# Hebbalali/dgp-toolbox

Measured on NVIDIA B200. Metric: DGP ELBO+grad point-samples/s, higher is better.
Workload: dtype f64

## Files before the change

### dgp_toolbox_b200/csrc/common.cuh

```cuda
#pragma once
#include <cuda_runtime.h>
#include <cstdint>
#include <type_traits>
#include <cstdio>
#include <string>

#define DGP_OK 0
#define DGP_ERR_CUDA -1
#define DGP_ERR_ARG -2
#define DGP_ERR_UNSUPPORTED -3
#define DGP_ERR_NUMERIC -4

namespace dgp {

constexpr int kTileM = 64;
constexpr int kTileP = 128;
constexpr int kMaxD = 32;

__host__ __device__ inline long round_up(long x, long m) { return (x + m - 1) / m * m; }

__device__ __forceinline__ void dmma884(double& c0, double& c1, double a, double b) {
  asm volatile("mma.sync.aligned.m8n8k4.row.col.f64.f64.f64.f64 {%0,%1},{%2},{%3},{%0,%1};"
               : "+d"(c0), "+d"(c1) : "d"(a), "d"(b));
}

__device__ __forceinline__ void cp_async16(void* smem, const void* gmem) {
  unsigned s = (unsigned)__cvta_generic_to_shared(smem);
  asm volatile("cp.async.cg.shared.global [%0], [%1], 16;" ::"r"(s), "l"(gmem));
}
__device__ __forceinline__ void cp_async8(void* smem, const void* gmem) {
  unsigned s = (unsigned)__cvta_generic_to_shared(smem);
  asm volatile("cp.async.ca.shared.global [%0], [%1], 8;" ::"r"(s), "l"(gmem));
}
__device__ __forceinline__ void cp_async_commit() { asm volatile("cp.async.commit_group;"); }
template <int N>
__device__ __forceinline__ void cp_async_wait() { asm volatile("cp.async.wait_group %0;" ::"n"(N)); }

__device__ __forceinline__ double exp_nonpos(double x) {
  const double xc = fmax(x, -700.0);
  double t = fma(xc, 1.4426950408889634074, 6755399441055744.0);
  const int n = __double2loint(t);
  t -= 6755399441055744.0;
  double r = fma(t, -6.93147180369123816490e-01, xc);
  r = fma(t, -1.90821492927058770002e-10, r);
  double p = 1.6059043836821613e-10;
  p = fma(p, r, 2.08767569878681e-09);
  p = fma(p, r, 2.505210838544172e-08);
  p = fma(p, r, 2.755731922398589e-07);
  p = fma(p, r, 2.7557319223985893e-06);
  p = fma(p, r, 2.48015873015873e-05);
  p = fma(p, r, 1.984126984126984e-04);
  p = fma(p, r, 1.388888888888889e-03);
  p = fma(p, r, 8.333333333333333e-03);
  p = fma(p, r, 4.1666666666666664e-02);
  p = fma(p, r, 1.6666666666666666e-01);
  p = fma(p, r, 0.5);
  p = fma(p, r, 1.0);
  p = fma(p, r, 1.0);
  const double y = __hiloint2double(__double2hiint(p) + (n << 20), __double2loint(p));
  return x != x ? x : y;
}

__device__ __forceinline__ void kernel_eval(int kind, double r2, double s2, double& k, double& gfac) {
  if (kind == 0) {
    k = s2 * exp_nonpos(-0.5 * r2);
    gfac = k;
  } else if (kind == 1) {
    const double a = 1.7320508075688772935;
    const double r = sqrt(fmax(r2, 1e-36)), e = exp_nonpos(-a * r);
    k = s2 * (1.0 + a * r) * e;
// ... 36 lines not shown
```

### dgp_toolbox_b200/csrc/dgp_b200.cu

```cuda
#include "../../include/dgp_b200.h"

#include <dlfcn.h>

#include <cmath>
#include <cstdlib>
#include <cstring>
#include <string>
#include <vector>

#include "acq.cuh"
#include "common.cuh"
#include "fused.cuh"
#include "fused_bwd.cuh"
#include "fullcov.cuh"
#include "extk.cuh"
#include "compkern.cuh"
#include "gemm.cuh"
#include "layer.cuh"
#include "philox.cuh"
#include "prep.cuh"
#include "small.cuh"

using namespace dgp;

// ... 284 lines not shown
    const long ctas = p.tiles * s;
    const long waves = (ctas + p.slots - 1) / p.slots;
    const double eff = (double)ctas / (double)(waves * p.slots);
    if (eff > best_eff + 0.02) { best_eff = eff; best = (int)s; }
  }
  return best;
}

template <typename F>
int dispatch_dmax(int D, F&& f) {
  if (D <= 1) return f(std::integral_constant<int, 1>());
  if (D <= 2) return f(std::integral_constant<int, 2>());
  if (D <= 4) return f(std::integral_constant<int, 4>());
  if (D <= 8) return f(std::integral_constant<int, 8>());
  if (D <= 16) return f(std::integral_constant<int, 16>());
  return f(std::integral_constant<int, 32>());
}

int check_layer(dgp_ctx* c, const dgp_layer_desc& L) {
  if (L.D_in < 1 || L.D_in > kMaxD - 1 || L.D_out < 1 || L.D_out > kMaxD || L.M < 1) {
    c->err = "layer widths must satisfy 1 <= D_in <= 31, 1 <= D_out <= 32, M >= 1";
    return DGP_ERR_ARG;
  }
  if (round_up(L.M, kTileM) > 768) { c->err = "M > 768 is not supported by the single-CTA Cholesky"; return DGP_ERR_UNSUPPORTED; }
  if (L.kernel_kind < 0 || L.kernel_kind > 2) { c->err = "kernel_kind must be 0 (SquaredExponential), 1 (Matern32) or 2 (Matern52)"; return DGP_ERR_UNSUPPORTED; }
  if (L.mean_kind < 0 || L.mean_kind > 2) { c->err = "mean_kind must be 0 (Zero), 1 (Identity) or 2 (Linear)"; return DGP_ERR_ARG; }
  if (L.mean_kind == 1 && L.D_in != L.D_out) { c->err = "Identity mean function needs D_in == D_out"; return DGP_ERR_ARG; }
  if (L.mean_kind == 2 && !L.mf_W) { c->err = "Linear mean function needs mf_W"; return DGP_ERR_ARG; }
  if (!L.Z || !L.lengthscales || !L.variance || !L.q_mu || !L.q_sqrt) { c->err = "null parameter pointer in layer descriptor"; return DGP_ERR_ARG; }
  return DGP_OK;
}

struct LayerWs {
  int M = 0, Mp = 0, D_in = 0, D_out = 0;
  double *Ku = nullptr, *Knj = nullptr, *L = nullptr, *Linv = nullptr, *LinvT = nullptr;
  double *RpT = nullptr, *Rcat = nullptr, *qmuP = nullptr;
  double *Kinv = nullptr, *alpha = nullptr, *KRcat = nullptr, *LRcat = nullptr, *KSK = nullptr;
  double *dKu = nullptr, *dR = nullptr, *dqmu = nullptr, *H = nullptr, *rbf_red = nullptr, *sgv = nullptr;
  double *dZk = nullptr, *kuu_part = nullptr, *kuu_red = nullptr, *kl = nullptr;
  double *Zs = nullptr, *zz = nullptr, *stream = nullptr;
  PanelDesc* sched = nullptr;
  int NP = 0, fcfg = -1;
  bool vform = false;
  bool white = false;
  double *Cmat = nullptr, *betaP = nullptr;
  double *CTcat = nullptr, *G1 = nullptr, *DCt = nullptr, *Wacc = nullptr, *dbeta = nullptr, *dqmu2 = nullptr, *dRcat = nullptr;
  double *dLinv = nullptr, *sq1 = nullptr, *sq2 = nullptr;
  double* bstream = nullptr; int bcfg = -1, NPb = 0;
  double* part_small = nullptr;
};

struct FusedChoice { int BM, PT; };
constexpr FusedChoice kFusedChoices[4] = {{128, 64}, {128, 32}, {64, 64}, {64, 32}};
constexpr size_t kMaxSmem = 227 * 1024;

size_t fused_smem(int cfg, int Mp, int D_in, int D_out) {
  switch (cfg) {
    case 0: return FusedCfg<128, 64, 4, 2>::smem_bytes(Mp, D_in, D_out);
    case 1: return FusedCfg<128, 32, 4, 2>::smem_bytes(Mp, D_in, D_out);
    case 2: return FusedCfg<64, 64, 2, 4>::smem_bytes(Mp, D_in, D_out);
    default: return FusedCfg<64, 32, 2, 4>::smem_bytes(Mp, D_in, D_out);
  }
}

int pick_fused_cfg(int Mp, int D_in, int D_out) {
  static const char* force = getenv("DGP_B200_FUSED_CFG");
  if (force) { const int cfg = atoi(force); if (cfg >= 0 && cfg < 4 && Mp % kFusedChoices[cfg].BM == 0 && fused_smem(cfg, Mp, D_in, D_out) <= kMaxSmem) return cfg; }
  for (int cfg = 0; cfg < 4; ++cfg) {
    if (Mp % kFusedChoices[cfg].BM) continue;
    if (fused_smem(cfg, Mp, D_in, D_out) <= kMaxSmem) return cfg;
  }
  return -1;
}

constexpr int kFusedBwdBM[2] = {128, 64};
size_t fused_bwd_smem(int cfg, int Mp, int D_in, int D_out) {
  return cfg == 0 ? FusedBwdCfg<128, 64, 4, 2>::smem_bytes(Mp, D_in, D_out) : FusedBwdCfg<64, 64, 2, 4>::smem_bytes(Mp, D_in, D_out);
}
int pick_fused_bwd_cfg(int Mp, int D_in, int D_out) {
  if (D_in > 16) return -1;
  static const char* force = getenv("DGP_B200_FUSED_BWD_CFG");
  for (int cfg = force ? atoi(force) : 0; cfg < 2; ++cfg) {
    if (cfg < 0 || Mp % kFusedBwdBM[cfg]) continue;
    if (fused_bwd_smem(cfg, Mp, D_in, D_out) <= kMaxSmem) return cfg;
  }
  return -1;
}

std::vector<PanelDesc> build_schedule(int Mp, int BM, int D_out, bool vform) {
  std::vector<PanelDesc> v;
  const int nb = Mp / BM, kpb = BM / kPanelK, kt = Mp / kPanelK;
  for (int i = nb - 1; i >= 0; --i)
    for (int ks = 0; ks < (i + 1) * kpb; ++ks) {
      int fl = (ks == 0 ? kPanelFirst : 0) | (ks == (i + 1) * kpb - 1 ? kPanelLast : 0) | (ks * kPanelK >= i * BM ? kPanelClip : 0);
      if ((fl & kPanelLast) && i == 0) fl |= kPanelStageEnd;
      v.push_back(PanelDesc{0, 0, i, ks * kPanelK, fl, 0});
    }
  auto upper = [&](int kind, int d0, int nd) {
    for (int i = 0; i < nb; ++i)
      for (int ks = i * kpb; ks < kt; ++ks) {
        int fl = (ks == i * kpb ? kPanelFirst : 0) | (ks == kt - 1 ? kPanelLast : 0) | (ks * kPanelK < (i + 1) * BM ? kPanelClip : 0);
        if ((fl & kPanelLast) && i == nb - 1) fl |= kPanelStageEnd;
        for (int d = d0; d < d0 + nd; ++d) v.push_back(PanelDesc{kind, d, i, ks * kPanelK, fl, 0});
      }
  };
  if (!vform) upper(1, 0, 1);
  for (int dp = 0; dp < D_out / 2; ++dp) upper(2, 2 * dp, 2);
  if (D_out & 1) upper(2, D_out - 1, 1);
  return v;
}

enum PrepLevel { PREP_FWD = 0, PREP_KL = 1, PREP_GRAD = 2 };

struct LayerPath { bool fused, vform; };

LayerPath ctx_path(const dgp_ctx* c, PrepLevel level, long point_samples) {
  const bool vform = level == PREP_FWD ? c->vform_forward_calls
                                       : level == PREP_GRAD && c->use_vform_grad && point_samples >= c->vform_grad_min_ps;
  return {c->use_fused, vform};
}

int chol_smem_optin(dgp_ctx* c) {
  if (c->chol_configured) return DGP_OK;
  CK(cudaFuncSetAttribute(chol_inv_kernel, cudaFuncAttributeMaxDynamicSharedMemorySize, (int)chol_smem_bytes(768)));
  CK(cudaFuncSetAttribute(tri_inv_kernel, cudaFuncAttributeMaxDynamicSharedMemorySize, (int)tri_inv_smem_bytes(768)));
  c->chol_configured = true;
  return DGP_OK;
}

void split_long_k(GemmArgs& g, int D, double* part) {
// ... 333 lines not shown
  CAT(DGP_CAT_RBF_BWD);
  RbfBwdArgs r;
  memset(&r, 0, sizeof(r));
  r.W = W; r.A = A; r.gq = up.gq; r.Gbar = Gbar; r.Xin = cl.Xin; r.xmod = cl.xmod; r.Z = d.Z; r.ls = d.lengthscales;
  r.var = d.variance; r.M = w.M; r.Mp = w.Mp; r.D_in = w.D_in; r.P = P; r.Pp = Pp; r.Gm = up.Gm; r.D_out = w.D_out;
  r.mean_kind = d.mean_kind; r.mfW = d.mf_W; r.kind = d.kernel_kind; r.dXin = dXin; r.XaugPad = XaugPad; r.part = rbf_part;
  const bool small = Pp / 128 < 2L * c->num_sms && rbf_bwd_smem_bytes(w.M, w.D_in) <= kRbfBwdSmemMax;
  nb = small ? Pp / kRbfCols : Pp / 128;
  const size_t smem = small ? rbf_bwd_smem_bytes(w.M, w.D_in) : ((size_t)w.M * w.D_in + kMaxD + 32) * sizeof(double);
  return dispatch_dmax(w.D_in, [&](auto dm) -> int {
    constexpr int DM = decltype(dm)::value;
    if (small) {
      if (!c->dry) CK(cudaFuncSetAttribute((rbf_bwd2d_kernel<DM, VF>), cudaFuncAttributeMaxDynamicSharedMemorySize, (int)kRbfBwdSmemMax));
      LAUNCH((rbf_bwd2d_kernel<DM, VF>), (unsigned)nb, 256, smem, r);
    } else {
      if (!c->dry) CK(cudaFuncSetAttribute((rbf_bwd_kernel<DM, VF>), cudaFuncAttributeMaxDynamicSharedMemorySize, (int)kRbfBwdSmemMax));
      LAUNCH((rbf_bwd_kernel<DM, VF>), (unsigned)nb, 128, smem, r);
    }
    return DGP_OK;
  });
}

int backward_layer(dgp_ctx* c, const dgp_layer_desc& d, const LayerWs& w, const ChunkLayer& cl, const Temps& tmp,
                   const Upstream& up, double* dXin, double* XaugPad, double* rbf_part, const ParamScratch& ps, long Nc, long S, bool first_chunk,
                   bool params = true) {
  const long P = Nc * S, Pp = round_up(P, kTileP);
  const int Mp = w.Mp, D = w.D_out;
  const double beta = first_chunk ? 0.0 : 1.0;
  double* dA = tmp.t0;
  double* W = tmp.t1;
  double* Gbar = tmp.t2;
  if (w.vform) {
    const double* V = cl.A;
    double* dV = dA;
    double* Kbar = W;
    const bool fused_bwd = w.bcfg >= 0;
    const long ntile64 = Pp / 64;
    long nbv = 0;
    if (fused_bwd) {
      CAT(DGP_CAT_FUSED_BWD);
      FusedBwdArgs f;
      memset(&f, 0, sizeof(f));
      f.stream = w.bstream; f.V = V; f.T = cl.T; f.GvT = up.GvT; f.gq = up.gq; f.Gm = up.GmPad; f.gm_ld = 32; f.beta = w.betaP;
      f.Zs = w.Zs; f.zz = w.zz; f.ls = d.lengthscales; f.var = d.variance; f.Xin = cl.Xin; f.xmod = cl.xmod; f.D_in = w.D_in;
      f.mfW = d.mf_W; f.mean_kind = d.mean_kind; f.kind = d.kernel_kind; f.M = w.M; f.Mp = Mp; f.D_out = D; f.P = P; f.Pp = Pp;
      f.dV = nullptr;
      f.Gbar = Gbar; f.dXin = dXin; f.XaugPad = XaugPad; f.part = rbf_part;
      f.warp_major_groups = c->warp_major_groups ? 1 : 0; f.group_skew = c->group_skew;
      nbv = ntile64 * (w.bcfg == 0 ? 2 : 4);
      const size_t smem = fused_bwd_smem(w.bcfg, Mp, w.D_in, D);
      const unsigned grid = (unsigned)(ntile64 < c->num_sms ? ntile64 : c->num_sms);
#define FUSED_BWD_LAUNCH(BM_, WM_, WN_, DM_)                                                                                \
      do {                                                                                                                  \
        if (!c->dry) CK(cudaFuncSetAttribute((fused_backward_kernel<BM_, 64, WM_, WN_, DM_>), cudaFuncAttributeMaxDynamicSharedMemorySize, (int)kMaxSmem)); \
        LAUNCH((fused_backward_kernel<BM_, 64, WM_, WN_, DM_>), grid, 384, smem, f);                                        \
      } while (0)
      if (w.bcfg == 0) { if (w.D_in <= 8) FUSED_BWD_LAUNCH(128, 4, 2, 8); else FUSED_BWD_LAUNCH(128, 4, 2, 16); }
      else { if (w.D_in <= 8) FUSED_BWD_LAUNCH(64, 2, 4, 8); else FUSED_BWD_LAUNCH(64, 2, 4, 16); }
#undef FUSED_BWD_LAUNCH
    } else {
    CAT(DGP_CAT_GEMM_BWD_DATA);
    GemmArgs g = gargs(w.betaP, 32, up.GmPad, 32, dV, Pp, Mp, (int)Pp, 32);
    RC(gemm(c, g, true));
    g = gargs(w.CTcat, (long)D * Mp, cl.T, Pp, dV, Pp, Mp, (int)Pp, D * Mp);
    g.a_tri = 1; g.kblocks = D; g.kblk = Mp; g.bscale = up.GvT; g.ld_bscale = Pp; g.bscale_mul = 2.0; g.beta = 1.0;
    if (D == 1) g.kblocks = 1;
    g.epi_plane = V; g.ld_epi = Pp; g.epi_col = up.gq; g.epi_mul = 2.0;
    RC(gemm(c, g, false));
    g = gargs(w.LinvT, Mp, dV, Pp, Kbar, Pp, Mp, (int)Pp, Mp);
    g.a_tri = 2;
    RC(gemm(c, g, false));
    RC(kernel_adjoint<true>(c, d, w, cl, up, Kbar, nullptr, Gbar, dXin, XaugPad, rbf_part, P, nbv));
    }
    if (!params) return DGP_OK;
    CAT(DGP_CAT_GEMM_BWD_PARAM);
    GemmArgs pg[3];
    const bool pnt[3] = {true, false, false};
    const int slots[3] = {1, 2, 3};
    pg[0] = gargs(V, Pp, V, Pp, w.Wacc, (long)D * Mp, Mp, Mp, (int)Pp);
    pg[0].alpha = 2.0; pg[0].beta = beta; pg[0].batch = D; pg[0].sA = 0; pg[0].sB = 0; pg[0].sC = Mp; pg[0].c_lower = 1;
    pg[0].kscale = up.GvT; pg[0].sScale = Pp;
    pg[1] = gargs(V, Pp, up.GmPad, 32, w.dbeta, 32, Mp, 32, (int)Pp);
    pg[1].beta = beta;
    pg[2] = gargs(Gbar, Pp, XaugPad, 32, w.H, 32, Mp, 32, (int)Pp);
    pg[2].beta = beta;
    RC(param_gemms(c, pg, pnt, 3, ps, slots, [&]() -> int {
      LAUNCH(reduce_partials_kernel, w.D_in + 1, 256, 0, rbf_part, nbv, w.D_in + 1, w.rbf_red, first_chunk ? 0 : 1);
      LAUNCH(reduce_partials_kernel, 3, 256, 0, up.part, up.nblocks, 3, w.sgv, first_chunk ? 0 : 1);
      return DGP_OK;
    }));
    return DGP_OK;
  }
  CAT(DGP_CAT_GEMM_BWD_DATA);
  RC(aform_adjoint(c, w, cl.T, up.GmPad, up.GvT, dA, W, Pp, &ps));
  long nb = 0;
  RC(kernel_adjoint<false>(c, d, w, cl, up, W, cl.A, Gbar, dXin, XaugPad, rbf_part, P, nb));
  if (!params) return DGP_OK;
  CAT(DGP_CAT_GEMM_BWD_PARAM);
  GemmArgs pg[4];
  const bool pnt[4] = {kAformParamNT[0], kAformParamNT[1], kAformParamNT[2], false};
  aform_param_args(w, W, cl.A, cl.T, up.GvT, up.GmPad, Pp, beta, pg);
  pg[3] = gargs(Gbar, Pp, XaugPad, 32, w.H, 32, Mp, 32, (int)Pp);
  pg[3].beta = beta;
  RC(param_gemms(c, pg, pnt, 4, ps, nullptr, [&]() -> int {
    LAUNCH(reduce_partials_kernel, w.D_in + 1, 256, 0, rbf_part, nb, w.D_in + 1, w.rbf_red, first_chunk ? 0 : 1);
    LAUNCH(reduce_partials_kernel, 3, 256, 0, up.part, up.nblocks, 3, w.sgv, first_chunk ? 0 : 1);
    return DGP_OK;
  }));
// ... 1565 lines not shown
```

### dgp_toolbox_b200/csrc/fused_bwd.cuh

```cuda
#pragma once
#include "common.cuh"
#include "fused.cuh"

namespace dgp {

struct FusedBwdArgs {
  const double* stream;
  const double* V; const double* T;
  const double* GvT; const double* gq;
  const double* Gm; int gm_ld;
  const double* beta;
  const double* Zs; const double* ls; const double* var;
  const double* Xin; long xmod; int D_in;
  const double* mfW; int mean_kind; int kind;
  int M, Mp, D_out; long P, Pp;
  double* dV; double* Gbar;
  double* dXin;
  double* XaugPad;
  double* part;
  int warp_major_groups, group_skew;
  const double* zz;
};

__host__ __device__ __forceinline__ int zigzag(int idx, int n) { return (idx & 1) ? n - 1 - (idx >> 1) : (idx >> 1); }

template <int BM>
__global__ void __launch_bounds__(256) pack_bwd_stream_kernel(const double* __restrict__ Cmat, const double* __restrict__ LinvT,
                                                              int Mp, int D, double* __restrict__ stream) {
  const int nb = Mp / BM, kpb = BM / kPanelK;
  int q = blockIdx.x, pass = 0, i = 0, d = 0, ks = 0;
  const int NP0 = D * kpb * nb * (nb + 1) / 2;
  if (q < NP0) {
    for (i = 0;; ++i) { const int cnt = D * (i + 1) * kpb; if (q < cnt) break; q -= cnt; }
    d = q / ((i + 1) * kpb); ks = zigzag(q % ((i + 1) * kpb), (i + 1) * kpb);
  } else {
    q -= NP0; pass = 1;
    for (i = 0;; ++i) { const int cnt = (nb - i) * kpb; if (q < cnt) break; q -= cnt; }
    ks = i * kpb + zigzag(q, (nb - i) * kpb);
  }
  double* dst = stream + (long)blockIdx.x * BM * kPanelK;
  for (int idx = threadIdx.x; idx < BM * kPanelK; idx += blockDim.x) {
    const int r = idx % BM, k = idx / BM;
    const int row = i * BM + r, col = ks * kPanelK + k;
    dst[panel_swz(r, k)] = pass == 0 ? Cmat[((long)d * Mp + col) * Mp + row] : LinvT[(long)row * Mp + col];
  }
}

template <int LO, int HI, int TM, int TN, int WM, int LDT, bool SC>
__device__ __forceinline__ void bwd_panel_block(double (&c0)[TM][TN], double (&c1)[TM][TN], const double* __restrict__ pan,
                                                const double* __restrict__ bt, const double (&sc)[TN], int wm, int g8, int t4) {
#pragma unroll
  for (int kk = 0; kk < 4; ++kk) {
    double bv[TN], av[HI - LO > 0 ? HI - LO : 1];
#pragma unroll
    for (int j = 0; j < TN; ++j) bv[j] = bt[kk * 4 * LDT + j * 8];
#pragma unroll
    for (int i = LO; i < HI; ++i) {
      const int row = i * 8 * WM + wm * 8 + g8;
      av[i - LO] = pan[row * kPanelK + (((kk ^ (row & 3)) << 2) | t4)];
    }
    if (SC) {
#pragma unroll
      for (int j = 0; j < TN; ++j) bv[j] *= sc[j];
    }
#pragma unroll
    for (int i = LO; i < HI; ++i)
#pragma unroll
      for (int j = 0; j < TN; ++j) dmma884(c0[i][j], c1[i][j], av[i - LO], bv[j]);
  }
}
template <int TM, int TN, int WM, int LDT, bool SC>
__device__ __forceinline__ void bwd_panel_dispatch(double (&c0)[TM][TN], double (&c1)[TM][TN], const double* pan, const double* bt,
                                                   const double (&sc)[TN], int wm, int g8, int t4, int lo, int hi) {
  static_assert(TM <= 4, "dispatch covers TM <= 4");
  if (lo == 0) {
    if (hi == TM) { bwd_panel_block<0, TM, TM, TN, WM, LDT, SC>(c0, c1, pan, bt, sc, wm, g8, t4); return; }
    if constexpr (TM >= 2) { if (hi == 1) { bwd_panel_block<0, 1, TM, TN, WM, LDT, SC>(c0, c1, pan, bt, sc, wm, g8, t4); return; } }
    if constexpr (TM >= 3) { if (hi == 2) { bwd_panel_block<0, 2, TM, TN, WM, LDT, SC>(c0, c1, pan, bt, sc, wm, g8, t4); return; } }
    if constexpr (TM >= 4) { if (hi == 3) { bwd_panel_block<0, 3, TM, TN, WM, LDT, SC>(c0, c1, pan, bt, sc, wm, g8, t4); return; } }
    return;
  }
  if constexpr (TM >= 2) { if (lo == TM - 1) { bwd_panel_block<TM - 1, TM, TM, TN, WM, LDT, SC>(c0, c1, pan, bt, sc, wm, g8, t4); return; } }
  if constexpr (TM >= 3) { if (lo == TM - 2) { bwd_panel_block<TM - 2, TM, TM, TN, WM, LDT, SC>(c0, c1, pan, bt, sc, wm, g8, t4); return; } }
  if constexpr (TM >= 4) { if (lo == TM - 3) { bwd_panel_block<TM - 3, TM, TM, TN, WM, LDT, SC>(c0, c1, pan, bt, sc, wm, g8, t4); return; } }
}



template <int BM, int PT, int WM, int WN>
struct FusedBwdCfg {
  static_assert(WM * WN == 8, "8 consumer warps");
  static constexpr int THREADS = 384;
  static constexpr int GT = WM * 32, GC = PT / WN;
  static constexpr int TM = BM / (8 * WM), TN = GC / 8;
  static constexpr int LDT = PT + 4;
  static constexpr int PANEL = BM * kPanelK, SLAB = kPanelK * LDT, STAGE = PANEL + SLAB;
  static constexpr int STAGES = 3;
  static size_t smem_bytes(int Mp, int D_in, int D_out) {
    return ((size_t)STAGES * STAGE + (size_t)Mp * LDT + (size_t)D_in * PT + (size_t)D_out * PT + (size_t)PT + 2 * STAGES + 2 + (size_t)WN * WM * (kMaxD + 1) + (size_t)PT * (D_in + 1)) * sizeof(double);
  }
};

template <int BM, int PT, int WM, int WN, int DMAX>
__global__ void __launch_bounds__(384, 1) fused_backward_kernel(FusedBwdArgs a) {
  using Cfg = FusedBwdCfg<BM, PT, WM, WN>;
  constexpr int TM = Cfg::TM, TN = Cfg::TN, LDT = Cfg::LDT, PANEL = Cfg::PANEL, STAGE = Cfg::STAGE, STAGES = Cfg::STAGES;
  constexpr int GT = Cfg::GT, GC = Cfg::GC, KPB = BM / kPanelK;
  constexpr int XSW = GC == 32 ? 1 : 0;
  extern __shared__ __align__(128) double bsmem[];
  double* pbuf = bsmem;
  double* tile = pbuf + STAGES * STAGE;
  double* xs_all = tile + (size_t)a.Mp * LDT;
  double* gv2_all = xs_all + a.D_in * PT;
  double* gq_all = gv2_all + a.D_out * PT;
  unsigned long long* full = reinterpret_cast<unsigned long long*>(gq_all + PT);
  unsigned long long* empty = full + STAGES;
  unsigned long long* vbar = empty + STAGES;
  double* red_all = reinterpret_cast<double*>(vbar + 2);
  double* us_all = red_all + WN * WM * (kMaxD + 1);

  const int tid = threadIdx.x, lane = tid & 31, warp = tid >> 5;
  const int nb = a.Mp / BM, kt = a.Mp / kPanelK;
  const int ntiles = (int)(a.Pp / PT);
  const int my_tiles = (int)blockIdx.x < ntiles ? (ntiles - (int)blockIdx.x + (int)gridDim.x - 1) / (int)gridDim.x : 0;

  if (tid == 0) {
    for (int s = 0; s < STAGES; ++s) { mbar_init(full + s, 1); mbar_init(empty + s, 8); }
    mbar_init(vbar, 1);
    asm volatile("fence.mbarrier_init.release.cluster;" ::: "memory");
  }
  __syncthreads();

  if (warp >= 8) {
    regs_shrink();
    if (warp > 8) return;
    if (lane == 0) {
      int st = 0;
      unsigned ph = 0;
#ifndef DGP_BWD_AHEAD
#define DGP_BWD_AHEAD 8
#endif
      constexpr int kAhead = DGP_BWD_AHEAD;
      int f_tl = 0, f_i = 0, f_d = 0, f_ks = 0;
      auto prefetch_next = [&]() {
        if (f_tl >= my_tiles) return;
        const double* trow = a.T + ((long)f_d * a.Mp + (long)zigzag(f_ks, (f_i + 1) * KPB) * kPanelK) * a.Pp + (long)(blockIdx.x + f_tl * gridDim.x) * PT;
#pragma unroll 4
        for (int r = 0; r < kPanelK; ++r)
          asm volatile("cp.async.bulk.prefetch.L2.global [%0], %1;" ::"l"(trow + (long)r * a.Pp), "r"(PT * 8) : "memory");
        if (++f_ks == (f_i + 1) * KPB) { f_ks = 0; if (++f_d == a.D_out) { f_d = 0; if (++f_i == nb) { f_i = 0; ++f_tl; } } }
      };
      for (int q = 0; q < kAhead; ++q) prefetch_next();
      for (int tl = 0; tl < my_tiles; ++tl) {
        const long p0 = (long)(blockIdx.x + tl * gridDim.x) * PT;
        const double* src = a.stream;
        int issued = 0;
        for (int i = 0; i < nb; ++i)
          for (int d = 0; d < a.D_out; ++d)
            for (int ksi = 0; ksi < (i + 1) * KPB; ++ksi) {
              const int ks = zigzag(ksi, (i + 1) * KPB);
              mbar_wait(empty + st, ph ^ 1);
              if (issued++ == STAGES) {
                mbar_arrive_expect_tx(vbar, (unsigned)(a.Mp * PT * 8));
                for (int r = 0; r < a.Mp; ++r) bulk_g2s(tile + r * LDT, a.V + (long)r * a.Pp + p0, PT * 8, vbar);
              }
              double* dst = pbuf + st * STAGE;
#ifdef DGP_BWD_EXPERIMENT_NO_SLABS
              mbar_arrive_expect_tx(full + st, PANEL * 8);
              bulk_g2s(dst, src, PANEL * 8, full + st);
#else
              const int r0 = max(0, ks * kPanelK - i * BM);
              mbar_arrive_expect_tx(full + st, (unsigned)(((BM - r0) * kPanelK + kPanelK * PT) * 8));
              bulk_g2s(dst + r0 * kPanelK, src + r0 * kPanelK, (unsigned)((BM - r0) * kPanelK * 8), full + st);
              const double* trow = a.T + ((long)d * a.Mp + (long)ks * kPanelK) * a.Pp + p0;
#pragma unroll 4
              for (int r = 0; r < kPanelK; ++r) bulk_g2s(dst + PANEL + r * LDT, trow + (long)r * a.Pp, PT * 8, full + st);
#endif
              prefetch_next();
              src += PANEL;
              if (++st == STAGES) { st = 0; ph ^= 1; }
            }
        for (int i = 0; i < nb; ++i)
          for (int ksi = 0; ksi < kt - i * KPB; ++ksi) {
            const int ks = i * KPB + zigzag(ksi, kt - i * KPB);
            mbar_wait(empty + st, ph ^ 1);
            const int nr = min(BM, ks * kPanelK - i * BM + kPanelK);
            mbar_arrive_expect_tx(full + st, (unsigned)(nr * kPanelK * 8));
            bulk_g2s(pbuf + st * STAGE, src, (unsigned)(nr * kPanelK * 8), full + st);
            src += PANEL;
            if (++st == STAGES) { st = 0; ph ^= 1; }
          }
      }
    }
    return;
  }

  regs_grow();
  const int g8 = lane >> 2, t4 = lane & 3;
  const int wm = a.warp_major_groups ? warp % WM : warp / WN, wn = a.warp_major_groups ? warp / WM : warp % WN;
  const int tg = wm * 32 + lane;
  const int col0 = wn * GC;
  double* xs = xs_all + wn * a.D_in * GC;
  double* gv2 = gv2_all + wn * a.D_out * GC;
  double* gqs = gq_all + wn * GC;
  double* red = red_all + wn * WM * (kMaxD + 1);
  double* us = us_all + wn * GC * (a.D_in + 1);
  const int bar_id = 1 + wn;
  const double s2 = a.var[0];
  int cst = 0;
  unsigned cph = 0;
  double c0[TM][TN], c1[TM][TN];

  if (a.group_skew > 0 && wn > 0) {
    const long long t0 = clock64();
    while (clock64() - t0 < (long long)a.group_skew * wn) {}
  }
#ifdef DGP_DEBUG_PHASECLK
  long long ph_pro = 0, ph_p0 = 0, ph_be = 0, ph_p1 = 0, ph_row = 0, ph_red = 0, ph_out = 0, ph_wait = 0;
  const long long ph_t0 = clock64();
#endif
  for (int tl = 0; tl < my_tiles; ++tl) {
    const long tile_index = (long)blockIdx.x + (long)tl * gridDim.x;
    const long p0 = tile_index * PT + col0;
    PH_MARK(ph_a);
    group_sync(bar_id, GT);
    for (int idx = tg; idx < a.D_in * GC; idx += GT) {
      const int j = idx / GC, c = idx % GC;
      const long p = p0 + c;
      xs[j * GC + (c ^ (XSW * ((j & 3) << 3)))] = (p < a.P) ? a.Xin[(p % a.xmod) * a.D_in + j] * (1.0 / a.ls[j]) : 0.0;
    }
    for (int idx = tg; idx < a.D_out * GC; idx += GT) {
      const int d = idx / GC, c = idx % GC;
      gv2[idx] = 2.0 * a.GvT[(long)d * a.Pp + p0 + c];
    }
    if (tg < GC) gqs[tg] = a.gq[p0 + tg];
    group_sync(bar_id, GT);

    PH_ADD(ph_pro, ph_a);
    for (int i = 0; i < nb; ++i) {
      PH_MARK(ph_b);
#pragma unroll
      for (int ti = 0; ti < TM; ++ti)
#pragma unroll
        for (int j = 0; j < TN; ++j) { c0[ti][j] = 0.0; c1[ti][j] = 0.0; }
      for (int d = 0; d < a.D_out; ++d) {
        double sc[TN];
#pragma unroll
        for (int j = 0; j < TN; ++j) sc[j] = gv2[d * GC + j * 8 + g8];
        for (int ksi = 0; ksi < (i + 1) * KPB; ++ksi) {
          const int ks = zigzag(ksi, (i + 1) * KPB);
          const int num = ks * kPanelK - i * BM - 7 - wm * 8;
          const int lo = num > 0 ? (num + 8 * WM - 1) / (8 * WM) : 0;
          const double* stage = pbuf + cst * STAGE;
          PH_MARK(ph_w);
          mbar_wait(full + cst, cph);
          PH_ADD(ph_wait, ph_w);
          bwd_panel_dispatch<TM, TN, WM, LDT, true>(c0, c1, stage, stage + PANEL + t4 * LDT + col0 + g8, sc, wm, g8, t4, lo < TM ? lo : 0, lo < TM ? TM : 0);
          __syncwarp();
          if (lane == 0) mbar_arrive(empty + cst);
          if (++cst == STAGES) { cst = 0; cph ^= 1; }
        }
      }
      PH_ADD(ph_p0, ph_b);
      PH_MARK(ph_c);
      for (int d = 0; d < a.D_out; d += 2) {
        const bool two = d + 1 < a.D_out;
        double gm0[2][TN], gm1[2][TN], bq[2][TM];
#pragma unroll
        for (int j = 0; j < TN; ++j) {
          const double* g = a.Gm + (p0 + j * 8 + 2 * t4) * a.gm_ld + d;
          gm0[0][j] = g[0]; gm1[0][j] = g[a.gm_ld];
          gm0[1][j] = two ? g[1] : 0.0; gm1[1][j] = two ? g[a.gm_ld + 1] : 0.0;
        }
#pragma unroll
        for (int ti = 0; ti < TM; ++ti) {
          const double* b = a.beta + (long)(i * BM + ti * 8 * WM + wm * 8 + g8) * 32 + d;
          bq[0][ti] = b[0]; bq[1][ti] = two ? b[1] : 0.0;
        }
#pragma unroll
        for (int u = 0; u < 2; ++u)
#pragma unroll
          for (int ti = 0; ti < TM; ++ti)
#pragma unroll
            for (int j = 0; j < TN; ++j) { c0[ti][j] = fma(bq[u][ti], gm0[u][j], c0[ti][j]); c1[ti][j] = fma(bq[u][ti], gm1[u][j], c1[ti][j]); }
      }
      if (i == 0) mbar_wait(vbar, (unsigned)(tl & 1));
#pragma unroll
      for (int ti = 0; ti < TM; ++ti) {
        const int row = i * BM + ti * 8 * WM + wm * 8 + g8;
#pragma unroll
        for (int j = 0; j < TN; ++j) {
          const int cl = j * 8 + 2 * t4;
          double2* tp = reinterpret_cast<double2*>(tile + row * LDT + col0 + cl);
          const double2 v = *tp;
          const double r0 = fma(2.0 * v.x, gqs[cl], c0[ti][j]), r1 = fma(2.0 * v.y, gqs[cl + 1], c1[ti][j]);
          *tp = make_double2(r0, r1);
          if (a.dV) *reinterpret_cast<double2*>(a.dV + (long)row * a.Pp + p0 + cl) = make_double2(r0, r1);
        }
      }
      PH_ADD(ph_be, ph_c);
    }
    PH_MARK(ph_d);
    group_sync(bar_id, GT);

    const double sc1[TN] = {};
    for (int i = 0; i < nb; ++i) {
#pragma unroll
      for (int ti = 0; ti < TM; ++ti)
#pragma unroll
        for (int j = 0; j < TN; ++j) { c0[ti][j] = 0.0; c1[ti][j] = 0.0; }
      for (int ksi = 0; ksi < kt - i * KPB; ++ksi) {
        const int ks = i * KPB + zigzag(ksi, kt - i * KPB);
        const int num = ks * kPanelK - i * BM + kPanelK - 1 - wm * 8;
        const int hi = num >= 0 ? min(TM, num / (8 * WM) + 1) : 0;
        const double* stage = pbuf + cst * STAGE;
        mbar_wait(full + cst, cph);
        bwd_panel_dispatch<TM, TN, WM, LDT, false>(c0, c1, stage, tile + (ks * kPanelK + t4) * LDT + col0 + g8, sc1, wm, g8, t4, 0, hi);
        __syncwarp();
        if (lane == 0) mbar_arrive(empty + cst);
        if (++cst == STAGES) { cst = 0; cph ^= 1; }
      }
      group_sync(bar_id, GT);
#pragma unroll
      for (int ti = 0; ti < TM; ++ti)
#pragma unroll
        for (int j = 0; j < TN; ++j) {
          const int row = i * BM + ti * 8 * WM + wm * 8 + g8, col = col0 + j * 8 + 2 * t4;
          *reinterpret_cast<double2*>(tile + row * LDT + col) = make_double2(c0[ti][j], c1[ti][j]);
        }
      group_sync(bar_id, GT);
    }

    PH_ADD(ph_p1, ph_d);
    PH_MARK(ph_e);
    constexpr int TNG = GC / 8, KS = DMAX / 4, NTJ = DMAX / 8 + 1, KC = GC / 4, MB = 4;
    const int J = a.D_in + 1, nmt = a.Mp / 8;
    double ds2 = 0.0, dla[NTJ - 1][2];
#pragma unroll
    for (int jt = 0; jt < NTJ - 1; ++jt) { dla[jt][0] = 0.0; dla[jt][1] = 0.0; }
    {
      double xx0[TNG], xx1[TNG], bx[KS][TNG];
#pragma unroll
      for (int nt = 0; nt < TNG; ++nt) {
        const int col = nt * 8 + 2 * t4;
        double q0 = 0.0, q1 = 0.0;
        for (int j = 0; j < a.D_in; ++j) {
          const int sw = XSW * ((j & 3) << 3);
          const double v0 = xs[j * GC + (col ^ sw)], v1 = xs[j * GC + ((col + 1) ^ sw)];
          q0 = fma(v0, v0, q0); q1 = fma(v1, v1, q1);
        }
        xx0[nt] = q0; xx1[nt] = q1;
      }
#pragma unroll
      for (int kk = 0; kk < KS; ++kk) {
        const int j = kk * 4 + t4;
#pragma unroll
        for (int nt = 0; nt < TNG; ++nt) bx[kk][nt] = j < a.D_in ? xs[j * GC + ((nt * 8 + g8) ^ (XSW * (t4 << 3)))] : 0.0;
      }
      auto sweep = [&](auto kconst) {
        constexpr int KIND = decltype(kconst)::value;
        for (int mt0 = wm; mt0 < nmt; mt0 += WM * MB) {
          double av[MB][KS], zzv[MB];
#pragma unroll
          for (int u = 0; u < MB; ++u) {
            const int m = (mt0 + u * WM) * 8 + g8;
            const bool ml = mt0 + u * WM < nmt && m < a.M;
#pragma unroll
            for (int kk = 0; kk < KS; ++kk) {
              const int j = kk * 4 + t4;
              av[u][kk] = (ml && j < a.D_in) ? a.Zs[(long)m * a.D_in + j] : 0.0;
            }
            zzv[u] = ml ? a.zz[m] : 0.0;
          }
// ... 192 lines not shown
```

Measured before the change: 6.318 million.

## Reverse fused backward row-block order and borrow V tile space as extra pipeline stages

The fused backward kernel now walks pass-0 row blocks from last to first. Not-yet-loaded V rows of the tile serve as extra ring stages, so the producer can run deeper ahead, and V is loaded per row block ("parked") through two alternating barriers instead of all at once. When D_out is even and the ring is deep enough, consumers process two output dims per panel step, which pairs the MMAs and halves the waits per panel. The stream packer is updated to match the new panel order. This adds complex ring and parity bookkeeping and more mbarriers, and ordering bugs could hang the kernel or corrupt results.

```diff
diff --git a/dgp_toolbox_b200/csrc/common.cuh b/dgp_toolbox_b200/csrc/common.cuh
--- a/dgp_toolbox_b200/csrc/common.cuh
+++ b/dgp_toolbox_b200/csrc/common.cuh
@@ -16,6 +16,7 @@
 constexpr int kTileM = 64;
 constexpr int kTileP = 128;
 constexpr int kMaxD = 32;
+constexpr size_t kMaxSmem = 227 * 1024;
 
 __host__ __device__ inline long round_up(long x, long m) { return (x + m - 1) / m * m; }
 
diff --git a/dgp_toolbox_b200/csrc/dgp_b200.cu b/dgp_toolbox_b200/csrc/dgp_b200.cu
--- a/dgp_toolbox_b200/csrc/dgp_b200.cu
+++ b/dgp_toolbox_b200/csrc/dgp_b200.cu
@@ -360,7 +360,6 @@
 
 struct FusedChoice { int BM, PT; };
 constexpr FusedChoice kFusedChoices[4] = {{128, 64}, {128, 32}, {64, 64}, {64, 32}};
-constexpr size_t kMaxSmem = 227 * 1024;
 
 size_t fused_smem(int cfg, int Mp, int D_in, int D_out) {
   switch (cfg) {
@@ -383,7 +382,7 @@
 
 constexpr int kFusedBwdBM[2] = {128, 64};
 size_t fused_bwd_smem(int cfg, int Mp, int D_in, int D_out) {
-  return cfg == 0 ? FusedBwdCfg<128, 64, 4, 2>::smem_bytes(Mp, D_in, D_out) : FusedBwdCfg<64, 64, 2, 4>::smem_bytes(Mp, D_in, D_out);
+  return cfg == 0 ? FusedBwdCfg<128, kFusedBwdPT, 4, 2>::smem_bytes(Mp, D_in, D_out) : FusedBwdCfg<64, kFusedBwdPT, 2, 4>::smem_bytes(Mp, D_in, D_out);
 }
 int pick_fused_bwd_cfg(int Mp, int D_in, int D_out) {
   if (D_in > 16) return -1;
@@ -823,8 +822,8 @@
       const unsigned grid = (unsigned)(ntile64 < c->num_sms ? ntile64 : c->num_sms);
 #define FUSED_BWD_LAUNCH(BM_, WM_, WN_, DM_)                                                                                \
       do {                                                                                                                  \
-        if (!c->dry) CK(cudaFuncSetAttribute((fused_backward_kernel<BM_, 64, WM_, WN_, DM_>), cudaFuncAttributeMaxDynamicSharedMemorySize, (int)kMaxSmem)); \
-        LAUNCH((fused_backward_kernel<BM_, 64, WM_, WN_, DM_>), grid, 384, smem, f);                                        \
+        if (!c->dry) CK(cudaFuncSetAttribute((fused_backward_kernel<BM_, kFusedBwdPT, WM_, WN_, DM_>), cudaFuncAttributeMaxDynamicSharedMemorySize, (int)kMaxSmem)); \
+        LAUNCH((fused_backward_kernel<BM_, kFusedBwdPT, WM_, WN_, DM_>), grid, 384, smem, f);                                        \
       } while (0)
       if (w.bcfg == 0) { if (w.D_in <= 8) FUSED_BWD_LAUNCH(128, 4, 2, 8); else FUSED_BWD_LAUNCH(128, 4, 2, 16); }
       else { if (w.D_in <= 8) FUSED_BWD_LAUNCH(64, 2, 4, 8); else FUSED_BWD_LAUNCH(64, 2, 4, 16); }
diff --git a/dgp_toolbox_b200/csrc/fused_bwd.cuh b/dgp_toolbox_b200/csrc/fused_bwd.cuh
--- a/dgp_toolbox_b200/csrc/fused_bwd.cuh
+++ b/dgp_toolbox_b200/csrc/fused_bwd.cuh
@@ -1,8 +1,13 @@
 #pragma once
 #include "common.cuh"
 #include "fused.cuh"
+#ifdef DGP_DEBUG_RING
+#include <cassert>
+#endif
 
 namespace dgp {
+
+constexpr int kFusedBwdPT = 64;
 
 struct FusedBwdArgs {
   const double* stream;
@@ -24,15 +29,84 @@
 
 __host__ __device__ __forceinline__ int zigzag(int idx, int n) { return (idx & 1) ? n - 1 - (idx >> 1) : (idx >> 1); }
 
+template <int BM, int PT>
+struct BwdRing {
+  static constexpr int LDT = PT + 4, PANEL = BM * kPanelK, SLAB = kPanelK * LDT, STAGE = PANEL + SLAB;
+  static constexpr int STAGES = 3, KPB = BM / kPanelK;
+  __host__ __device__ static constexpr int extra(int i) { return i * BM * LDT / STAGE; }
+  __host__ __device__ static constexpr int depth(int i) { return STAGES + extra(i); }
+  __host__ __device__ static constexpr bool paired(int i, int D_out) {
+#ifdef DGP_BWD_EXPERIMENT_NO_PAIR
+    return false;
+#else
+    return D_out % 2 == 0 && depth(i) >= 4;
+#endif
+  }
+  static constexpr int NSTAGE_MAX = depth(((int)(kMaxSmem / sizeof(double)) - STAGES * STAGE) / LDT / BM - 1);
+  static_assert(BM * LDT >= STAGE, "every row block borrows at least one stage more than the next lower one (the V parks rely on it)");
+  static_assert(KPB > STAGES, "the first row block of a tile holds more panels than the own stages");
+  static_assert(NSTAGE_MAX <= 32, "one phase bit per stage in an unsigned");
+};
+
+__host__ __device__ __forceinline__ void bwd_p0_panel(int q, int nk, bool paired, int& d, int& ks) {
+  int ksi;
+  if (paired) { const int r = q % (2 * nk); d = 2 * (q / (2 * nk)) + (r & 1); ksi = r >> 1; }
+  else { d = q / nk; ksi = q % nk; }
+  ks = zigzag(ksi, nk);
+}
+
+struct BwdRingPos {
+  int s = 0;
+  unsigned par = 0;
+  __host__ __device__ void enter(int R) { if (s >= R) s = 0; }
+  __host__ __device__ unsigned parity_of(int t) const { return (par >> t) & 1u; }
+  __host__ __device__ unsigned parity() const { return parity_of(s); }
+  __host__ __device__ void next(int R) { par ^= 1u << s; if (++s == R) s = 0; }
+};
+
+template <class Ring, class Fill, class Release, class Park>
+__host__ __device__ __forceinline__ void bwd_tile_schedule(int nb, int D_out, BwdRingPos& w, Fill&& fill, Release&& release, Park&& park) {
+  constexpr int KPB = Ring::KPB;
+  w.s = 0;
+  int issued = 0;
+  for (int i = nb - 1; i >= 0; --i) {
+    const int R = Ring::depth(i), nk = (i + 1) * KPB;
+    const bool pr = Ring::paired(i, D_out);
+    w.enter(R);
+    for (int q = 0; q < D_out * nk; ++q) {
+      if (i < nb - 1 && q == R) {
+        for (int t = R; t < Ring::depth(i + 1); ++t) release(t, w.parity_of(t) ^ 1u);
+        park(i);
+      }
+      if (issued++ == Ring::STAGES) {
+        release(0, w.parity_of(0) ^ 1u);
+        park(nb - 1);
+      }
+      int d, ks;
+      bwd_p0_panel(q, nk, pr, d, ks);
+      fill(w.s, w.parity() ^ 1u, 0, i, d, ks);
+      w.next(R);
+    }
+  }
+  w.enter(Ring::STAGES);
+  const int kt = nb * KPB;
+  for (int i = 0; i < nb; ++i)
+    for (int ksi = 0; ksi < kt - i * KPB; ++ksi) {
+      fill(w.s, w.parity() ^ 1u, 1, i, 0, i * KPB + zigzag(ksi, kt - i * KPB));
+      w.next(Ring::STAGES);
+    }
+}
+
 template <int BM>
 __global__ void __launch_bounds__(256) pack_bwd_stream_kernel(const double* __restrict__ Cmat, const double* __restrict__ LinvT,
                                                               int Mp, int D, double* __restrict__ stream) {
+  using Ring = BwdRing<BM, kFusedBwdPT>;
   const int nb = Mp / BM, kpb = BM / kPanelK;
   int q = blockIdx.x, pass = 0, i = 0, d = 0, ks = 0;
   const int NP0 = D * kpb * nb * (nb + 1) / 2;
   if (q < NP0) {
-    for (i = 0;; ++i) { const int cnt = D * (i + 1) * kpb; if (q < cnt) break; q -= cnt; }
-    d = q / ((i + 1) * kpb); ks = zigzag(q % ((i + 1) * kpb), (i + 1) * kpb);
+    for (i = nb - 1;; --i) { const int cnt = D * (i + 1) * kpb; if (q < cnt) break; q -= cnt; }
+    bwd_p0_panel(q, (i + 1) * kpb, Ring::paired(i, D), d, ks);
   } else {
     q -= NP0; pass = 1;
     for (i = 0;; ++i) { const int cnt = (nb - i) * kpb; if (q < cnt) break; q -= cnt; }
@@ -85,19 +159,54 @@
   if constexpr (TM >= 4) { if (lo == TM - 3) { bwd_panel_block<TM - 3, TM, TM, TN, WM, LDT, SC>(c0, c1, pan, bt, sc, wm, g8, t4); return; } }
 }
 
-
+template <int LO, int HI, int TM, int TN, int WM, int LDT>
+__device__ __forceinline__ void bwd_panel_block2(double (&c0)[TM][TN], double (&c1)[TM][TN], const double* __restrict__ panA,
+                                                 const double* __restrict__ panB, const double* __restrict__ btA,
+                                                 const double* __restrict__ btB, const double (&sa)[TN], const double (&sb)[TN],
+                                                 int wm, int g8, int t4) {
+#pragma unroll
+  for (int kk = 0; kk < 4; ++kk) {
+    double ba[TN], bb[TN], aa[HI - LO], ab[HI - LO];
+#pragma unroll
+    for (int j = 0; j < TN; ++j) { ba[j] = btA[kk * 4 * LDT + j * 8]; bb[j] = btB[kk * 4 * LDT + j * 8]; }
+#pragma unroll
+    for (int i = LO; i < HI; ++i) {
+      const int row = i * 8 * WM + wm * 8 + g8;
+      const int off = row * kPanelK + (((kk ^ (row & 3)) << 2) | t4);
+      aa[i - LO] = panA[off];
+      ab[i - LO] = panB[off];
+    }
+#pragma unroll
+    for (int j = 0; j < TN; ++j) { ba[j] *= sa[j]; bb[j] *= sb[j]; }
+#pragma unroll
+    for (int i = LO; i < HI; ++i)
+#pragma unroll
+      for (int j = 0; j < TN; ++j) dmma884(c0[i][j], c1[i][j], aa[i - LO], ba[j]);
+#pragma unroll
+    for (int i = LO; i < HI; ++i)
+#pragma unroll
+      for (int j = 0; j < TN; ++j) dmma884(c0[i][j], c1[i][j], ab[i - LO], bb[j]);
+  }
+}
+template <int TM, int TN, int WM, int LDT>
+__device__ __forceinline__ void bwd_panel_dispatch2(double (&c0)[TM][TN], double (&c1)[TM][TN], const double* panA, const double* panB,
+                                                    const double* btA, const double* btB, const double (&sa)[TN], const double (&sb)[TN],
+                                                    int wm, int g8, int t4, int lo) {
+  if (lo == 0) { bwd_panel_block2<0, TM, TM, TN, WM, LDT>(c0, c1, panA, panB, btA, btB, sa, sb, wm, g8, t4); return; }
+  if constexpr (TM >= 2) { if (lo == TM - 1) { bwd_panel_block2<TM - 1, TM, TM, TN, WM, LDT>(c0, c1, panA, panB, btA, btB, sa, sb, wm, g8, t4); return; } }
+  if constexpr (TM >= 3) { if (lo == TM - 2) { bwd_panel_block2<TM - 2, TM, TM, TN, WM, LDT>(c0, c1, panA, panB, btA, btB, sa, sb, wm, g8, t4); return; } }
+  if constexpr (TM >= 4) { if (lo == TM - 3) { bwd_panel_block2<TM - 3, TM, TM, TN, WM, LDT>(c0, c1, panA, panB, btA, btB, sa, sb, wm, g8, t4); return; } }
+}
 
 template <int BM, int PT, int WM, int WN>
-struct FusedBwdCfg {
+struct FusedBwdCfg : BwdRing<BM, PT> {
+  using Ring = BwdRing<BM, PT>;
   static_assert(WM * WN == 8, "8 consumer warps");
   static constexpr int THREADS = 384;
   static constexpr int GT = WM * 32, GC = PT / WN;
   static constexpr int TM = BM / (8 * WM), TN = GC / 8;
-  static constexpr int LDT = PT + 4;
-  static constexpr int PANEL = BM * kPanelK, SLAB = kPanelK * LDT, STAGE = PANEL + SLAB;
-  static constexpr int STAGES = 3;
   static size_t smem_bytes(int Mp, int D_in, int D_out) {
-    return ((size_t)STAGES * STAGE + (size_t)Mp * LDT + (size_t)D_in * PT + (size_t)D_out * PT + (size_t)PT + 2 * STAGES + 2 + (size_t)WN * WM * (kMaxD + 1) + (size_t)PT * (D_in + 1)) * sizeof(double);
+    return ((size_t)Ring::STAGES * Ring::STAGE + (size_t)Mp * Ring::LDT + (size_t)D_in * PT + (size_t)D_out * PT + (size_t)PT + 2 * Ring::NSTAGE_MAX + 2 + (size_t)WN * WM * (kMaxD + 1) + (size_t)PT * (D_in + 1)) * sizeof(double);
   }
 };
 
@@ -105,7 +214,7 @@
 __global__ void __launch_bounds__(384, 1) fused_backward_kernel(FusedBwdArgs a) {
   using Cfg = FusedBwdCfg<BM, PT, WM, WN>;
   constexpr int TM = Cfg::TM, TN = Cfg::TN, LDT = Cfg::LDT, PANEL = Cfg::PANEL, STAGE = Cfg::STAGE, STAGES = Cfg::STAGES;
-  constexpr int GT = Cfg::GT, GC = Cfg::GC, KPB = BM / kPanelK;
+  constexpr int GT = Cfg::GT, GC = Cfg::GC, KPB = BM / kPanelK, NSTAGE = Cfg::NSTAGE_MAX;
   constexpr int XSW = GC == 32 ? 1 : 0;
   extern __shared__ __align__(128) double bsmem[];
   double* pbuf = bsmem;
@@ -114,8 +223,8 @@
   double* gv2_all = xs_all + a.D_in * PT;
   double* gq_all = gv2_all + a.D_out * PT;
   unsigned long long* full = reinterpret_cast<unsigned long long*>(gq_all + PT);
-  unsigned long long* empty = full + STAGES;
-  unsigned long long* vbar = empty + STAGES;
+  unsigned long long* empty = full + NSTAGE;
+  unsigned long long* vbar = empty + NSTAGE;
   double* red_all = reinterpret_cast<double*>(vbar + 2);
   double* us_all = red_all + WN * WM * (kMaxD + 1);
 
@@ -125,8 +234,8 @@
   const int my_tiles = (int)blockIdx.x < ntiles ? (ntiles - (int)blockIdx.x + (int)gridDim.x - 1) / (int)gridDim.x : 0;
 
   if (tid == 0) {
-    for (int s = 0; s < STAGES; ++s) { mbar_init(full + s, 1); mbar_init(empty + s, 8); }
-    mbar_init(vbar, 1);
+    for (int s = 0; s < NSTAGE; ++s) { mbar_init(full + s, 1); mbar_init(empty + s, 8); }
+    mbar_init(vbar, 1); mbar_init(vbar + 1, 1);
     asm volatile("fence.mbarrier_init.release.cluster;" ::: "memory");
   }
   __syncthreads();
@@ -135,61 +244,59 @@
     regs_shrink();
     if (warp > 8) return;
     if (lane == 0) {
-      int st = 0;
-      unsigned ph = 0;
+      BwdRingPos w;
+      unsigned vk = 0;
 #ifndef DGP_BWD_AHEAD
 #define DGP_BWD_AHEAD 8
 #endif
       constexpr int kAhead = DGP_BWD_AHEAD;
-      int f_tl = 0, f_i = 0, f_d = 0, f_ks = 0;
+      int f_tl = 0, f_i = nb - 1, f_q = 0;
       auto prefetch_next = [&]() {
         if (f_tl >= my_tiles) return;
-        const double* trow = a.T + ((long)f_d * a.Mp + (long)zigzag(f_ks, (f_i + 1) * KPB) * kPanelK) * a.Pp + (long)(blockIdx.x + f_tl * gridDim.x) * PT;
+        const int nk = (f_i + 1) * KPB;
+        int d, ks;
+        bwd_p0_panel(f_q, nk, Cfg::paired(f_i, a.D_out), d, ks);
+        const double* trow = a.T + ((long)d * a.Mp + (long)ks * kPanelK) * a.Pp + (long)(blockIdx.x + f_tl * gridDim.x) * PT;
 #pragma unroll 4
         for (int r = 0; r < kPanelK; ++r)
           asm volatile("cp.async.bulk.prefetch.L2.global [%0], %1;" ::"l"(trow + (long)r * a.Pp), "r"(PT * 8) : "memory");
-        if (++f_ks == (f_i + 1) * KPB) { f_ks = 0; if (++f_d == a.D_out) { f_d = 0; if (++f_i == nb) { f_i = 0; ++f_tl; } } }
+        if (++f_q == a.D_out * nk) { f_q = 0; if (--f_i < 0) { f_i = nb - 1; ++f_tl; } }
       };
       for (int q = 0; q < kAhead; ++q) prefetch_next();
       for (int tl = 0; tl < my_tiles; ++tl) {
         const long p0 = (long)(blockIdx.x + tl * gridDim.x) * PT;
         const double* src = a.stream;
-        int issued = 0;
-        for (int i = 0; i < nb; ++i)
-          for (int d = 0; d < a.D_out; ++d)
-            for (int ksi = 0; ksi < (i + 1) * KPB; ++ksi) {
-              const int ks = zigzag(ksi, (i + 1) * KPB);
-              mbar_wait(empty + st, ph ^ 1);
-              if (issued++ == STAGES) {
-                mbar_arrive_expect_tx(vbar, (unsigned)(a.Mp * PT * 8));
-                for (int r = 0; r < a.Mp; ++r) bulk_g2s(tile + r * LDT, a.V + (long)r * a.Pp + p0, PT * 8, vbar);
-              }
-              double* dst = pbuf + st * STAGE;
+        auto fill = [&](int s, unsigned parity, int pass, int i, int d, int ks) {
+          mbar_wait(empty + s, parity);
+          double* dst = pbuf + s * STAGE;
+          if (pass == 0) {
 #ifdef DGP_BWD_EXPERIMENT_NO_SLABS
-              mbar_arrive_expect_tx(full + st, PANEL * 8);
-              bulk_g2s(dst, src, PANEL * 8, full + st);
+            mbar_arrive_expect_tx(full + s, PANEL * 8);
+            bulk_g2s(dst, src, PANEL * 8, full + s);
 #else
-              const int r0 = max(0, ks * kPanelK - i * BM);
-              mbar_arrive_expect_tx(full + st, (unsigned)(((BM - r0) * kPanelK + kPanelK * PT) * 8));
-              bulk_g2s(dst + r0 * kPanelK, src + r0 * kPanelK, (unsigned)((BM - r0) * kPanelK * 8), full + st);
-              const double* trow = a.T + ((long)d * a.Mp + (long)ks * kPanelK) * a.Pp + p0;
+            const int r0 = max(0, ks * kPanelK - i * BM);
+            mbar_arrive_expect_tx(full + s, (unsigned)(((BM - r0) * kPanelK + kPanelK * PT) * 8));
+            bulk_g2s(dst + r0 * kPanelK, src + r0 * kPanelK, (unsigned)((BM - r0) * kPanelK * 8), full + s);
+            const double* trow = a.T + ((long)d * a.Mp + (long)ks * kPanelK) * a.Pp + p0;
 #pragma unroll 4
-              for (int r = 0; r < kPanelK; ++r) bulk_g2s(dst + PANEL + r * LDT, trow + (long)r * a.Pp, PT * 8, full + st);
+            for (int r = 0; r < kPanelK; ++r) bulk_g2s(dst + PANEL + r * LDT, trow + (long)r * a.Pp, PT * 8, full + s);
 #endif
-              prefetch_next();
-              src += PANEL;
-              if (++st == STAGES) { st = 0; ph ^= 1; }
-            }
-        for (int i = 0; i < nb; ++i)
-          for (int ksi = 0; ksi < kt - i * KPB; ++ksi) {
-            const int ks = i * KPB + zigzag(ksi, kt - i * KPB);
-            mbar_wait(empty + st, ph ^ 1);
+            prefetch_next();
+          } else {
             const int nr = min(BM, ks * kPanelK - i * BM + kPanelK);
-            mbar_arrive_expect_tx(full + st, (unsigned)(nr * kPanelK * 8));
-            bulk_g2s(pbuf + st * STAGE, src, (unsigned)(nr * kPanelK * 8), full + st);
-            src += PANEL;
-            if (++st == STAGES) { st = 0; ph ^= 1; }
-          }
+            mbar_arrive_expect_tx(full + s, (unsigned)(nr * kPanelK * 8));
+            bulk_g2s(dst, src, (unsigned)(nr * kPanelK * 8), full + s);
+          }
+          src += PANEL;
+        };
+        auto release = [&](int s, unsigned parity) { mbar_wait(empty + s, parity); };
+        auto park = [&](int i) {
+          unsigned long long* vb = vbar + (vk & 1);
+          mbar_arrive_expect_tx(vb, (unsigned)(BM * PT * 8));
+          for (int r = i * BM; r < (i + 1) * BM; ++r) bulk_g2s(tile + r * LDT, a.V + (long)r * a.Pp + p0, PT * 8, vb);
+          ++vk;
+        };
+        bwd_tile_schedule<typename Cfg::Ring>(nb, a.D_out, w, fill, release, park);
       }
     }
     return;
@@ -207,8 +314,8 @@
   double* us = us_all + wn * GC * (a.D_in + 1);
   const int bar_id = 1 + wn;
   const double s2 = a.var[0];
-  int cst = 0;
-  unsigned cph = 0;
+  BwdRingPos cw;
+  unsigned vk = 0;
   double c0[TM][TN], c1[TM][TN];
 
   if (a.group_skew > 0 && wn > 0) {
@@ -237,28 +344,64 @@
     group_sync(bar_id, GT);
 
     PH_ADD(ph_pro, ph_a);
-    for (int i = 0; i < nb; ++i) {
+    cw.s = 0;
+    for (int i = nb - 1; i >= 0; --i) {
       PH_MARK(ph_b);
+      const int R = Cfg::depth(i), nk = (i + 1) * KPB;
+      cw.enter(R);
+#ifdef DGP_DEBUG_RING
+      assert((R - STAGES) * STAGE <= i * BM * LDT);
+#endif
 #pragma unroll
       for (int ti = 0; ti < TM; ++ti)
 #pragma unroll
         for (int j = 0; j < TN; ++j) { c0[ti][j] = 0.0; c1[ti][j] = 0.0; }
-      for (int d = 0; d < a.D_out; ++d) {
-        double sc[TN];
-#pragma unroll
-        for (int j = 0; j < TN; ++j) sc[j] = gv2[d * GC + j * 8 + g8];
-        for (int ksi = 0; ksi < (i + 1) * KPB; ++ksi) {
-          const int ks = zigzag(ksi, (i + 1) * KPB);
-          const int num = ks * kPanelK - i * BM - 7 - wm * 8;
-          const int lo = num > 0 ? (num + 8 * WM - 1) / (8 * WM) : 0;
-          const double* stage = pbuf + cst * STAGE;
-          PH_MARK(ph_w);
-          mbar_wait(full + cst, cph);
-          PH_ADD(ph_wait, ph_w);
-          bwd_panel_dispatch<TM, TN, WM, LDT, true>(c0, c1, stage, stage + PANEL + t4 * LDT + col0 + g8, sc, wm, g8, t4, lo < TM ? lo : 0, lo < TM ? TM : 0);
-          __syncwarp();
-          if (lane == 0) mbar_arrive(empty + cst);
-          if (++cst == STAGES) { cst = 0; cph ^= 1; }
+      if (Cfg::paired(i, a.D_out)) {
+        for (int d = 0; d < a.D_out; d += 2) {
+          double sa[TN], sb[TN];
+#pragma unroll
+          for (int j = 0; j < TN; ++j) { sa[j] = gv2[d * GC + j * 8 + g8]; sb[j] = gv2[(d + 1) * GC + j * 8 + g8]; }
+          for (int ksi = 0; ksi < nk; ++ksi) {
+            const int ks = zigzag(ksi, nk);
+            const int num = ks * kPanelK - i * BM - 7 - wm * 8;
+            const int lo = num > 0 ? (num + 8 * WM - 1) / (8 * WM) : 0;
+            const int sA = cw.s;
+            const unsigned pA = cw.parity();
+            cw.next(R);
+            const int sB = cw.s;
+            const unsigned pB = cw.parity();
+            cw.next(R);
+            const double* stA = pbuf + sA * STAGE;
+            const double* stB = pbuf + sB * STAGE;
+            PH_MARK(ph_w);
+            mbar_wait(full + sA, pA);
+            mbar_wait(full + sB, pB);
+            PH_ADD(ph_wait, ph_w);
+            if (lo < TM)
+              bwd_panel_dispatch2<TM, TN, WM, LDT>(c0, c1, stA, stB, stA + PANEL + t4 * LDT + col0 + g8, stB + PANEL + t4 * LDT + col0 + g8,
+                                                   sa, sb, wm, g8, t4, lo);
+            __syncwarp();
+            if (lane == 0) { mbar_arrive(empty + sA); mbar_arrive(empty + sB); }
+          }
+        }
+      } else {
+        for (int d = 0; d < a.D_out; ++d) {
+          double sc[TN];
+#pragma unroll
+          for (int j = 0; j < TN; ++j) sc[j] = gv2[d * GC + j * 8 + g8];
+          for (int ksi = 0; ksi < nk; ++ksi) {
+            const int ks = zigzag(ksi, nk);
+            const int num = ks * kPanelK - i * BM - 7 - wm * 8;
+            const int lo = num > 0 ? (num + 8 * WM - 1) / (8 * WM) : 0;
+            const double* stage = pbuf + cw.s * STAGE;
+            PH_MARK(ph_w);
+            mbar_wait(full + cw.s, cw.parity());
+            PH_ADD(ph_wait, ph_w);
+            bwd_panel_dispatch<TM, TN, WM, LDT, true>(c0, c1, stage, stage + PANEL + t4 * LDT + col0 + g8, sc, wm, g8, t4, lo < TM ? lo : 0, lo < TM ? TM : 0);
+            __syncwarp();
+            if (lane == 0) mbar_arrive(empty + cw.s);
+            cw.next(R);
+          }
         }
       }
       PH_ADD(ph_p0, ph_b);
@@ -284,7 +427,8 @@
 #pragma unroll
             for (int j = 0; j < TN; ++j) { c0[ti][j] = fma(bq[u][ti], gm0[u][j], c0[ti][j]); c1[ti][j] = fma(bq[u][ti], gm1[u][j], c1[ti][j]); }
       }
-      if (i == 0) mbar_wait(vbar, (unsigned)(tl & 1));
+      mbar_wait(vbar + (vk & 1), (vk >> 1) & 1u);
+      ++vk;
 #pragma unroll
       for (int ti = 0; ti < TM; ++ti) {
         const int row = i * BM + ti * 8 * WM + wm * 8 + g8;
@@ -304,6 +448,7 @@
     group_sync(bar_id, GT);
 
     const double sc1[TN] = {};
+    cw.enter(STAGES);
     for (int i = 0; i < nb; ++i) {
 #pragma unroll
       for (int ti = 0; ti < TM; ++ti)
@@ -313,12 +458,12 @@
         const int ks = i * KPB + zigzag(ksi, kt - i * KPB);
         const int num = ks * kPanelK - i * BM + kPanelK - 1 - wm * 8;
         const int hi = num >= 0 ? min(TM, num / (8 * WM) + 1) : 0;
-        const double* stage = pbuf + cst * STAGE;
-        mbar_wait(full + cst, cph);
+        const double* stage = pbuf + cw.s * STAGE;
+        mbar_wait(full + cw.s, cw.parity());
         bwd_panel_dispatch<TM, TN, WM, LDT, false>(c0, c1, stage, tile + (ks * kPanelK + t4) * LDT + col0 + g8, sc1, wm, g8, t4, 0, hi);
         __syncwarp();
-        if (lane == 0) mbar_arrive(empty + cst);
-        if (++cst == STAGES) { cst = 0; cph ^= 1; }
+        if (lane == 0) mbar_arrive(empty + cw.s);
+        cw.next(STAGES);
       }
       group_sync(bar_id, GT);
 #pragma unroll
```

Result: slower. 6.107 million, median of 6 (-3.3%).
